# FoundationVision/OmniTokenizer

Measured on NVIDIA H100. Metric: video_frames_per_sec_encode_decode, higher is better.
Workload: dtype f32

## Files before the change

omnitokenizer_b200/csrc/attention_f16.cu:

```cuda
#include "omt_common.cuh"
#include "tc_ptx.cuh"
#include <cuda.h>

namespace omt {
int g_attn_f16_ctas = 2;
namespace af16 {
using namespace omt::ptx;

constexpr int QT = 128, KT = 64, D = 64;
constexpr int TILE = KT * D * 2;
constexpr int OFF_Q = 0;
constexpr int OFF_KV = 4 * TILE;
constexpr int OFF_P = OFF_KV + 8 * TILE;
constexpr int OFF_CTRL = OFF_P + 4 * TILE;
constexpr int SMEM = OFF_CTRL + 1024 + 1024;
constexpr int THREADS = 256;

struct Args {
  const float* vinv;
  long long rows;
  float* o; uint16_t* o_hi; uint16_t* o_lo; int ldo;
  int N;
  float scale_log2;
};

__global__ void __launch_bounds__(THREADS, 1)
attn_f16_kernel(const __grid_constant__ CUtensorMap tmQh, const __grid_constant__ CUtensorMap tmQl,
                const __grid_constant__ CUtensorMap tmKh, const __grid_constant__ CUtensorMap tmKl,
                const __grid_constant__ CUtensorMap tmVh, const __grid_constant__ CUtensorMap tmVl, const Args a) {
  extern __shared__ uint8_t smem_raw[];
  uint8_t* smem = smem_raw + ((1024u - (smem_u32(smem_raw) & 1023u)) & 1023u);
  uint64_t* bars = reinterpret_cast<uint64_t*>(smem + OFF_CTRL);
  uint64_t& q_full = bars[0];
  uint64_t* full = bars + 1;
  float* red = reinterpret_cast<float*>(smem + OFF_CTRL + 64);

  const int tid = threadIdx.x, warp = tid >> 5, lane = tid & 31;
  const int wg = warp >> 2, qd = lane & 3;
  const int qt = blockIdx.x, head = blockIdx.y, seq = blockIdx.z;
  const int ntiles = a.N / KT;
  const int row_q0 = seq * a.N + qt * QT;
  const int row_k0 = seq * a.N;
  const int col0 = head * D;

  if (tid == 0) {
    prefetch_map(&tmQh); prefetch_map(&tmQl); prefetch_map(&tmKh); prefetch_map(&tmKl); prefetch_map(&tmVh); prefetch_map(&tmVl);
    mbar_init(&q_full, 1); mbar_init(&full[0], 1); mbar_init(&full[1], 1);
    fence_barrier_init();
  }
  __syncthreads();
  pdl_sync();

  auto issue_kv = [&](int j) {
    const int s = j & 1;
    uint8_t* sp = smem + OFF_KV + s * 4 * TILE;
    const int kr = row_k0 + j * KT;
    mbar_expect_tx(&full[s], 4 * TILE);
    tma_load_2d(&tmKh, &full[s], sp, col0, kr);
    tma_load_2d(&tmKl, &full[s], sp + TILE, col0, kr);
    tma_load_2d(&tmVh, &full[s], sp + 2 * TILE, col0, kr);
    tma_load_2d(&tmVl, &full[s], sp + 3 * TILE, col0, kr);
  };
  if (tid == 0) {
    mbar_expect_tx(&q_full, 4 * TILE);
    for (int w = 0; w < 2; ++w) {
      tma_load_2d(&tmQh, &q_full, smem + OFF_Q + w * TILE, col0, row_q0 + w * 64);
      tma_load_2d(&tmQl, &q_full, smem + OFF_Q + (2 + w) * TILE, col0, row_q0 + w * 64);
    }
    issue_kv(0);
    if (ntiles > 1) issue_kv(1);
  }

  const float* vinv_h = a.vinv + (size_t)head * a.rows + row_k0;
  float vmx = 0.f;
  for (int i = tid; i < a.N; i += THREADS) vmx = fmaxf(vmx, __ldg(vinv_h + i));
  vmx = warp_max(vmx);
  if (lane == 0) red[warp] = vmx;
  __syncthreads();
#pragma unroll
  for (int i = 0; i < 8; ++i) vmx = fmaxf(vmx, red[i]);
  float p_scale, p_inv;
  row_scale(vmx, p_scale, p_inv);

  const uint32_t sb = smem_u32(smem);
  const uint64_t dq_hi = desc_sw128(sb + OFF_Q + wg * TILE), dq_lo = desc_sw128(sb + OFF_Q + (2 + wg) * TILE);
  const uint32_t p_hi = sb + OFF_P + wg * 2 * TILE, p_lo = p_hi + TILE;
  const uint64_t dp_hi = desc_sw128(p_hi), dp_lo = desc_sw128(p_lo);
  const int rl0 = (warp & 3) * 16 + (lane >> 2);
  float o_acc[32];
#pragma unroll
  for (int i = 0; i < 32; ++i) o_acc[i] = 0.f;
  float m_run[2] = {-INFINITY, -INFINITY}, l_run[2] = {0.f, 0.f};
  mbar_wait(&q_full, 0);

  for (int j = 0; j < ntiles; ++j) {
    const int s = j & 1;
    const uint32_t kv = sb + OFF_KV + s * 4 * TILE;
    mbar_wait(&full[s], (j >> 1) & 1);
    float sv[32];
    {
      const uint64_t dk_hi = desc_sw128(kv), dk_lo = desc_sw128(kv + TILE);
      wg_fence();
#pragma unroll
      for (int kk = 0; kk < 4; ++kk) {
        const uint64_t adv = (uint64_t)(kk * 2);
        wgmma_f16_n64(sv, dq_lo + adv, dk_hi + adv, kk != 0);
        wgmma_f16_n64(sv, dq_hi + adv, dk_lo + adv, 1);
        wgmma_f16_n64(sv, dq_hi + adv, dk_hi + adv, 1);
      }
      wg_commit();
      wg_wait<0>();
    }
    float alpha[2], nm[2];
#pragma unroll
    for (int h = 0; h < 2; ++h) {
      float mx = -INFINITY;
#pragma unroll
      for (int jj = 0; jj < 8; ++jj) mx = fmaxf(mx, fmaxf(sv[4 * jj + 2 * h], sv[4 * jj + 2 * h + 1]));
      mx = fmaxf(mx, __shfl_xor_sync(0xffffffffu, mx, 1));
      mx = fmaxf(mx, __shfl_xor_sync(0xffffffffu, mx, 2));
      const float m_new = fmaxf(m_run[h], mx);
      alpha[h] = ex2_fast((m_run[h] - m_new) * a.scale_log2);
      m_run[h] = m_new;
      nm[h] = -m_new;
    }
    const float* vi = vinv_h + j * KT;
    float ps[2] = {0.f, 0.f};
#pragma unroll
    for (int jj = 0; jj < 8; ++jj) {
      const int key = 8 * jj + 2 * qd;
      const float2 w = __ldg(reinterpret_cast<const float2*>(vi + key));
#pragma unroll
      for (int h = 0; h < 2; ++h) {
        const float e0 = ex2_fast((sv[4 * jj + 2 * h] + nm[h]) * a.scale_log2);
        const float e1 = ex2_fast((sv[4 * jj + 2 * h + 1] + nm[h]) * a.scale_log2);
        ps[h] += e0 + e1;
        uint32_t hw, lw;
        split2u(e0 * (w.x * p_scale), e1 * (w.y * p_scale), hw, lw);
        const int r = rl0 + 8 * h;
        const uint32_t off = (uint32_t)r * 128u + (uint32_t)((jj ^ (r & 7)) << 4) + (uint32_t)(qd * 4);
        asm volatile("st.shared.b32 [%0], %1;" ::"r"(p_hi + off), "r"(hw) : "memory");
        asm volatile("st.shared.b32 [%0], %1;" ::"r"(p_lo + off), "r"(lw) : "memory");
      }
    }
#pragma unroll
    for (int h = 0; h < 2; ++h) {
      l_run[h] = fmaf(l_run[h], alpha[h], ps[h]);
#pragma unroll
      for (int jj = 0; jj < 8; ++jj) { o_acc[4 * jj + 2 * h] *= alpha[h]; o_acc[4 * jj + 2 * h + 1] *= alpha[h]; }
    }
    fence_async_smem();
    wg_bar(1 + wg);
    {
      const uint32_t vh = kv + 2 * TILE, vl = kv + 3 * TILE;
      wg_fence();
#pragma unroll
      for (int kk = 0; kk < 4; ++kk) {
        const uint64_t adv = (uint64_t)(kk * 2);
        const uint64_t dvh = desc_sw128(vh + kk * 2048), dvl = desc_sw128(vl + kk * 2048);
        wgmma_f16_n64_tb(o_acc, dp_lo + adv, dvh, 1);
        wgmma_f16_n64_tb(o_acc, dp_hi + adv, dvl, 1);
        wgmma_f16_n64_tb(o_acc, dp_hi + adv, dvh, 1);
      }
      wg_commit();
      wg_wait<0>();
    }
    __syncthreads();
    if (tid == 0 && j + 2 < ntiles) issue_kv(j + 2);
  }
#pragma unroll
  for (int h = 0; h < 2; ++h) {
    float l = l_run[h];
    l += __shfl_xor_sync(0xffffffffu, l, 1);
    l += __shfl_xor_sync(0xffffffffu, l, 2);
    const float inv = p_inv / l;
    const size_t ooff = (size_t)(row_q0 + wg * 64 + rl0 + 8 * h) * a.ldo + col0 + 2 * qd;
#pragma unroll
    for (int jj = 0; jj < 8; ++jj) {
      const float2 ov = make_float2(o_acc[4 * jj + 2 * h] * inv, o_acc[4 * jj + 2 * h + 1] * inv);
      if (a.o_hi != nullptr) store_split2(a.o_hi, a.o_lo, ooff + 8 * jj, ov);
      else *reinterpret_cast<float2*>(a.o + ooff + 8 * jj) = ov;
    }
  }
}

typedef CUresult (*EncodeTiledFn)(CUtensorMap*, CUtensorMapDataType, cuuint32_t, void*, const cuuint64_t*,
                                  const cuuint64_t*, const cuuint32_t*, const cuuint32_t*, CUtensorMapInterleave,
                                  CUtensorMapSwizzle, CUtensorMapL2promotion, CUtensorMapFloatOOBfill);

static int encode2d(CUtensorMap* m, const uint16_t* base, int cols, long long rows, int ld) {
  static EncodeTiledFn fn = nullptr;
  if (fn == nullptr) {
    void* p = nullptr;
    cudaDriverEntryPointQueryResult qres;
    if (cudaGetDriverEntryPoint("cuTensorMapEncodeTiled", &p, cudaEnableDefault, &qres) == cudaSuccess &&
        qres == cudaDriverEntryPointSuccess)
      fn = reinterpret_cast<EncodeTiledFn>(p);
  }
  if (fn == nullptr) { set_error("cuTensorMapEncodeTiled entry point not found"); return OMT_E_CUDA; }
  cuuint64_t dims[2] = {(cuuint64_t)cols, (cuuint64_t)rows};
  cuuint64_t strides[1] = {(cuuint64_t)ld * 2};
  cuuint32_t box[2] = {64, (cuuint32_t)KT};
  cuuint32_t estr[2] = {1, 1};
  CUresult r = fn(m, CU_TENSOR_MAP_DATA_TYPE_FLOAT16, 2, const_cast<uint16_t*>(base), dims, strides, box, estr,
                  CU_TENSOR_MAP_INTERLEAVE_NONE, CU_TENSOR_MAP_SWIZZLE_128B, CU_TENSOR_MAP_L2_PROMOTION_L2_256B,
                  CU_TENSOR_MAP_FLOAT_OOB_FILL_NONE);
  if (r != CUDA_SUCCESS) { set_error("cuTensorMapEncodeTiled failed (%d)", (int)r); return OMT_E_CUDA; }
  return OMT_OK;
}

}
}

using namespace omt;

extern "C" int omt_attn_spatial_h(const uint16_t* q_hi, const uint16_t* q_lo, int ldq, const uint16_t* k_hi,
                                  const uint16_t* k_lo, int ldk, const uint16_t* v_hi, const uint16_t* v_lo, int ldv,
                                  const float* vinv, float qk_plane_scale, float* o, uint16_t* o_hi, uint16_t* o_lo, int ldo,
                                  int n_seq, int N, int heads, float scale, omt_stream_t stream) {
  using namespace af16;
  OMT_ENTER();
  OMT_REQUIRE(q_hi && q_lo && k_hi && k_lo && v_hi && v_lo && vinv && (o || o_hi) && ((o_hi == nullptr) == (o_lo == nullptr)),
              "omt_attn_spatial_h: null pointer");
  OMT_REQUIRE(N > 0 && N % QT == 0, "omt_attn_spatial_h: N=%d must be a multiple of 128", N);
  OMT_REQUIRE(ldq % 8 == 0 && ldk % 8 == 0 && ldv % 8 == 0 && ldo % 4 == 0, "omt_attn_spatial_h: bad leading dims");
  OMT_REQUIRE(((uintptr_t)q_hi | (uintptr_t)q_lo | (uintptr_t)k_hi | (uintptr_t)k_lo | (uintptr_t)v_hi | (uintptr_t)v_lo | (uintptr_t)vinv |
               (uintptr_t)o | (uintptr_t)o_hi | (uintptr_t)o_lo) % 16 == 0, "omt_attn_spatial_h: pointers must be 16-byte aligned");
  OMT_REQUIRE(heads > 0 && heads <= 65535 && n_seq <= 65535 && qk_plane_scale > 0.f, "omt_attn_spatial_h: bad arguments");
  if (n_seq == 0) return OMT_OK;
  const long long rows = (long long)n_seq * N;
  CUtensorMap tmQh, tmQl, tmKh, tmKl, tmVh, tmVl;
  int rc;
  if ((rc = encode2d(&tmQh, q_hi, heads * D, rows, ldq))) return rc;
  if ((rc = encode2d(&tmQl, q_lo, heads * D, rows, ldq))) return rc;
  if ((rc = encode2d(&tmKh, k_hi, heads * D, rows, ldk))) return rc;
  if ((rc = encode2d(&tmKl, k_lo, heads * D, rows, ldk))) return rc;
  if ((rc = encode2d(&tmVh, v_hi, heads * D, rows, ldv))) return rc;
  if ((rc = encode2d(&tmVl, v_lo, heads * D, rows, ldv))) return rc;
  static bool attr[64];
  int dev = 0;
  cudaGetDevice(&dev);
  if (dev >= 0 && dev < 64 && !attr[dev]) {
    OMT_CUDA(cudaFuncSetAttribute(attn_f16_kernel, cudaFuncAttributeMaxDynamicSharedMemorySize, SMEM));
    attr[dev] = true;
  }
  Args a{vinv, rows, o, o_hi, o_lo, ldo, N, scale * 1.4426950408889634f / qk_plane_scale};
  dim3 grid(N / QT, heads, n_seq);
  OMT_CUDA(launch_k(attn_f16_kernel, grid, dim3(THREADS), SMEM, (cudaStream_t)stream, tmQh, tmQl, tmKh, tmKl, tmVh, tmVl, a));
  OMT_LAUNCH_CHECK();
  return OMT_OK;
}
```

omnitokenizer_b200/csrc/tc_ptx.cuh:

```cuda
#pragma once
#include <cuda.h>
#include <cstdint>

namespace omt {
namespace ptx {

__device__ __forceinline__ uint32_t smem_u32(const void* p) { return static_cast<uint32_t>(__cvta_generic_to_shared(p)); }

__device__ __forceinline__ void mbar_init(uint64_t* bar, uint32_t count) {
  asm volatile("mbarrier.init.shared::cta.b64 [%0], %1;" ::"r"(smem_u32(bar)), "r"(count));
}
__device__ __forceinline__ void mbar_expect_tx(uint64_t* bar, uint32_t bytes) {
  asm volatile("mbarrier.arrive.expect_tx.shared::cta.b64 _, [%0], %1;" ::"r"(smem_u32(bar)), "r"(bytes) : "memory");
}
__device__ __forceinline__ void mbar_arrive(uint64_t* bar) {
  asm volatile("mbarrier.arrive.shared::cta.b64 _, [%0];" ::"r"(smem_u32(bar)) : "memory");
}
__device__ __forceinline__ void mbar_wait(uint64_t* bar, uint32_t parity) {
  const uint32_t addr = smem_u32(bar);
  const long long t0 = clock64();
  for (uint32_t it = 0;; ++it) {
    uint32_t ok;
    asm volatile(
        "{\n\t"
        ".reg .pred p;\n\t"
        "mbarrier.try_wait.parity.shared::cta.b64 p, [%1], %2;\n\t"
        "selp.b32 %0, 1, 0, p;\n\t"
        "}\n" : "=r"(ok) : "r"(addr), "r"(parity) : "memory");
    if (ok) break;
    if ((it & 0x3ff) == 0x3ff && clock64() - t0 > 4000000000LL) __trap();
  }
}
__device__ __forceinline__ void fence_barrier_init() { asm volatile("fence.mbarrier_init.release.cluster;" ::: "memory"); }

__device__ __forceinline__ uint32_t cluster_ctarank() { uint32_t r; asm volatile("mov.u32 %0, %%cluster_ctarank;" : "=r"(r)); return r; }
__device__ __forceinline__ uint32_t mapa(uint32_t addr, uint32_t rank) {
  uint32_t r;
  asm volatile("mapa.shared::cluster.u32 %0, %1, %2;" : "=r"(r) : "r"(addr), "r"(rank));
  return r;
}
__device__ __forceinline__ void cluster_arrive() { asm volatile("barrier.cluster.arrive.release.aligned;" ::: "memory"); }
__device__ __forceinline__ void cluster_wait() { asm volatile("barrier.cluster.wait.acquire.aligned;" ::: "memory"); }

template <uint32_t R> __device__ __forceinline__ void setmaxnreg_dec() { asm volatile("setmaxnreg.dec.sync.aligned.u32 %0;" ::"n"(R)); }
template <uint32_t R> __device__ __forceinline__ void setmaxnreg_inc() { asm volatile("setmaxnreg.inc.sync.aligned.u32 %0;" ::"n"(R)); }

__device__ __forceinline__ void tma_load_2d(const CUtensorMap* map, uint64_t* bar, void* dst, int c0, int c1) {
  asm volatile(
      "cp.async.bulk.tensor.2d.shared::cluster.global.tile.mbarrier::complete_tx::bytes [%0], [%1, {%3, %4}], [%2];"
      ::"r"(smem_u32(dst)), "l"(reinterpret_cast<uint64_t>(map)), "r"(smem_u32(bar)), "r"(c0), "r"(c1) : "memory");
}
__device__ __forceinline__ void tma_load_3d(const CUtensorMap* map, uint64_t* bar, void* dst, int c0, int c1, int c2) {
  asm volatile(
      "cp.async.bulk.tensor.3d.shared::cluster.global.tile.mbarrier::complete_tx::bytes [%0], [%1, {%3, %4, %5}], [%2];"
      ::"r"(smem_u32(dst)), "l"(reinterpret_cast<uint64_t>(map)), "r"(smem_u32(bar)), "r"(c0), "r"(c1), "r"(c2) : "memory");
}
__device__ __forceinline__ void prefetch_map(const CUtensorMap* map) {
  asm volatile("prefetch.tensormap [%0];" ::"l"(reinterpret_cast<uint64_t>(map)) : "memory");
}
__device__ __forceinline__ void fence_async_smem() { asm volatile("fence.proxy.async.shared::cta;" ::: "memory"); }
__device__ __forceinline__ void wg_bar(int id) { asm volatile("bar.sync %0, 128;" ::"r"(id) : "memory"); }
__device__ __forceinline__ void named_bar_sync(int id, int n) { asm volatile("bar.sync %0, %1;" ::"r"(id), "r"(n) : "memory"); }
__device__ __forceinline__ void named_bar_arrive(int id, int n) { asm volatile("bar.arrive %0, %1;" ::"r"(id), "r"(n) : "memory"); }

__device__ __forceinline__ float tf32_rn(float x) {
  return __uint_as_float((__float_as_uint(x) + 0x1000u) & 0xffffe000u);
}

__device__ __forceinline__ uint64_t desc_sw128(uint32_t saddr) {
  uint64_t d = 0;
  d |= (uint64_t)((saddr >> 4) & 0x3fff);
  d |= (uint64_t)1 << 16;
  d |= (uint64_t)(1024 >> 4) << 32;
  d |= (uint64_t)1 << 62;
  return d;
}
__device__ __forceinline__ void wg_fence() { asm volatile("wgmma.fence.sync.aligned;" ::: "memory"); }
__device__ __forceinline__ void wg_commit() { asm volatile("wgmma.commit_group.sync.aligned;" ::: "memory"); }
template <int N> __device__ __forceinline__ void wg_wait() { asm volatile("wgmma.wait_group.sync.aligned %0;" ::"n"(N) : "memory"); }

__device__ __forceinline__ void wgmma_tf32_n64(float (&d)[32], uint64_t da, uint64_t db, uint32_t scale_d) {
  asm volatile(
      "{\n\t.reg .pred p;\n\tsetp.ne.b32 p, %34, 0;\n\t"
      "wgmma.mma_async.sync.aligned.m64n64k8.f32.tf32.tf32 "
      "{%0, %1, %2, %3, %4, %5, %6, %7, %8, %9, %10, %11, %12, %13, %14, %15, %16, %17, %18, %19, %20, %21, %22, %23, %24, %25, %26, %27, %28, %29, %30, %31}, %32, %33, p, 1, 1;\n\t}\n"
      : "+f"(d[0]), "+f"(d[1]), "+f"(d[2]), "+f"(d[3]), "+f"(d[4]), "+f"(d[5]), "+f"(d[6]), "+f"(d[7]), "+f"(d[8]), "+f"(d[9]), "+f"(d[10]), "+f"(d[11]), "+f"(d[12]), "+f"(d[13]), "+f"(d[14]), "+f"(d[15]), "+f"(d[16]), "+f"(d[17]), "+f"(d[18]), "+f"(d[19]), "+f"(d[20]), "+f"(d[21]), "+f"(d[22]), "+f"(d[23]), "+f"(d[24]), "+f"(d[25]), "+f"(d[26]), "+f"(d[27]), "+f"(d[28]), "+f"(d[29]), "+f"(d[30]), "+f"(d[31])
      : "l"(da), "l"(db), "r"(scale_d));
}
__device__ __forceinline__ void wgmma_f16_n64(float (&d)[32], uint64_t da, uint64_t db, uint32_t scale_d) {
  asm volatile(
      "{\n\t.reg .pred p;\n\tsetp.ne.b32 p, %34, 0;\n\t"
      "wgmma.mma_async.sync.aligned.m64n64k16.f32.f16.f16 "
      "{%0, %1, %2, %3, %4, %5, %6, %7, %8, %9, %10, %11, %12, %13, %14, %15, %16, %17, %18, %19, %20, %21, %22, %23, %24, %25, %26, %27, %28, %29, %30, %31}, %32, %33, p, 1, 1, 0, 0;\n\t}\n"
      : "+f"(d[0]), "+f"(d[1]), "+f"(d[2]), "+f"(d[3]), "+f"(d[4]), "+f"(d[5]), "+f"(d[6]), "+f"(d[7]), "+f"(d[8]), "+f"(d[9]), "+f"(d[10]), "+f"(d[11]), "+f"(d[12]), "+f"(d[13]), "+f"(d[14]), "+f"(d[15]), "+f"(d[16]), "+f"(d[17]), "+f"(d[18]), "+f"(d[19]), "+f"(d[20]), "+f"(d[21]), "+f"(d[22]), "+f"(d[23]), "+f"(d[24]), "+f"(d[25]), "+f"(d[26]), "+f"(d[27]), "+f"(d[28]), "+f"(d[29]), "+f"(d[30]), "+f"(d[31])
      : "l"(da), "l"(db), "r"(scale_d));
}
__device__ __forceinline__ void wgmma_tf32_n128(float (&d)[64], uint64_t da, uint64_t db, uint32_t scale_d) {
  asm volatile(
      "{\n\t.reg .pred p;\n\tsetp.ne.b32 p, %66, 0;\n\t"
      "wgmma.mma_async.sync.aligned.m64n128k8.f32.tf32.tf32 "
      "{%0, %1, %2, %3, %4, %5, %6, %7, %8, %9, %10, %11, %12, %13, %14, %15, %16, %17, %18, %19, %20, %21, %22, %23, %24, %25, %26, %27, %28, %29, %30, %31, %32, %33, %34, %35, %36, %37, %38, %39, %40, %41, %42, %43, %44, %45, %46, %47, %48, %49, %50, %51, %52, %53, %54, %55, %56, %57, %58, %59, %60, %61, %62, %63}, %64, %65, p, 1, 1;\n\t}\n"
      : "+f"(d[0]), "+f"(d[1]), "+f"(d[2]), "+f"(d[3]), "+f"(d[4]), "+f"(d[5]), "+f"(d[6]), "+f"(d[7]), "+f"(d[8]), "+f"(d[9]), "+f"(d[10]), "+f"(d[11]), "+f"(d[12]), "+f"(d[13]), "+f"(d[14]), "+f"(d[15]), "+f"(d[16]), "+f"(d[17]), "+f"(d[18]), "+f"(d[19]), "+f"(d[20]), "+f"(d[21]), "+f"(d[22]), "+f"(d[23]), "+f"(d[24]), "+f"(d[25]), "+f"(d[26]), "+f"(d[27]), "+f"(d[28]), "+f"(d[29]), "+f"(d[30]), "+f"(d[31]), "+f"(d[32]), "+f"(d[33]), "+f"(d[34]), "+f"(d[35]), "+f"(d[36]), "+f"(d[37]), "+f"(d[38]), "+f"(d[39]), "+f"(d[40]), "+f"(d[41]), "+f"(d[42]), "+f"(d[43]), "+f"(d[44]), "+f"(d[45]), "+f"(d[46]), "+f"(d[47]), "+f"(d[48]), "+f"(d[49]), "+f"(d[50]), "+f"(d[51]), "+f"(d[52]), "+f"(d[53]), "+f"(d[54]), "+f"(d[55]), "+f"(d[56]), "+f"(d[57]), "+f"(d[58]), "+f"(d[59]), "+f"(d[60]), "+f"(d[61]), "+f"(d[62]), "+f"(d[63])
      : "l"(da), "l"(db), "r"(scale_d));
}
__device__ __forceinline__ void wgmma_f16_n128(float (&d)[64], uint64_t da, uint64_t db, uint32_t scale_d) {
  asm volatile(
      "{\n\t.reg .pred p;\n\tsetp.ne.b32 p, %66, 0;\n\t"
      "wgmma.mma_async.sync.aligned.m64n128k16.f32.f16.f16 "
      "{%0, %1, %2, %3, %4, %5, %6, %7, %8, %9, %10, %11, %12, %13, %14, %15, %16, %17, %18, %19, %20, %21, %22, %23, %24, %25, %26, %27, %28, %29, %30, %31, %32, %33, %34, %35, %36, %37, %38, %39, %40, %41, %42, %43, %44, %45, %46, %47, %48, %49, %50, %51, %52, %53, %54, %55, %56, %57, %58, %59, %60, %61, %62, %63}, %64, %65, p, 1, 1, 0, 0;\n\t}\n"
      : "+f"(d[0]), "+f"(d[1]), "+f"(d[2]), "+f"(d[3]), "+f"(d[4]), "+f"(d[5]), "+f"(d[6]), "+f"(d[7]), "+f"(d[8]), "+f"(d[9]), "+f"(d[10]), "+f"(d[11]), "+f"(d[12]), "+f"(d[13]), "+f"(d[14]), "+f"(d[15]), "+f"(d[16]), "+f"(d[17]), "+f"(d[18]), "+f"(d[19]), "+f"(d[20]), "+f"(d[21]), "+f"(d[22]), "+f"(d[23]), "+f"(d[24]), "+f"(d[25]), "+f"(d[26]), "+f"(d[27]), "+f"(d[28]), "+f"(d[29]), "+f"(d[30]), "+f"(d[31]), "+f"(d[32]), "+f"(d[33]), "+f"(d[34]), "+f"(d[35]), "+f"(d[36]), "+f"(d[37]), "+f"(d[38]), "+f"(d[39]), "+f"(d[40]), "+f"(d[41]), "+f"(d[42]), "+f"(d[43]), "+f"(d[44]), "+f"(d[45]), "+f"(d[46]), "+f"(d[47]), "+f"(d[48]), "+f"(d[49]), "+f"(d[50]), "+f"(d[51]), "+f"(d[52]), "+f"(d[53]), "+f"(d[54]), "+f"(d[55]), "+f"(d[56]), "+f"(d[57]), "+f"(d[58]), "+f"(d[59]), "+f"(d[60]), "+f"(d[61]), "+f"(d[62]), "+f"(d[63])
      : "l"(da), "l"(db), "r"(scale_d));
}
__device__ __forceinline__ void wgmma_f16_n64_tb(float (&d)[32], uint64_t da, uint64_t db, uint32_t scale_d) {
  asm volatile(
      "{\n\t.reg .pred p;\n\tsetp.ne.b32 p, %34, 0;\n\t"
      "wgmma.mma_async.sync.aligned.m64n64k16.f32.f16.f16 "
      "{%0, %1, %2, %3, %4, %5, %6, %7, %8, %9, %10, %11, %12, %13, %14, %15, %16, %17, %18, %19, %20, %21, %22, %23, %24, %25, %26, %27, %28, %29, %30, %31}, %32, %33, p, 1, 1, 0, 1;\n\t}\n"
      : "+f"(d[0]), "+f"(d[1]), "+f"(d[2]), "+f"(d[3]), "+f"(d[4]), "+f"(d[5]), "+f"(d[6]), "+f"(d[7]), "+f"(d[8]), "+f"(d[9]), "+f"(d[10]), "+f"(d[11]), "+f"(d[12]), "+f"(d[13]), "+f"(d[14]), "+f"(d[15]), "+f"(d[16]), "+f"(d[17]), "+f"(d[18]), "+f"(d[19]), "+f"(d[20]), "+f"(d[21]), "+f"(d[22]), "+f"(d[23]), "+f"(d[24]), "+f"(d[25]), "+f"(d[26]), "+f"(d[27]), "+f"(d[28]), "+f"(d[29]), "+f"(d[30]), "+f"(d[31])
      : "l"(da), "l"(db), "r"(scale_d));
}

}
}
```

Measured before the change: 3492.

## Warp-specialize attention into persistent producer/consumer pipeline with register-operand P

Rewrites the f16-split attention kernel as a persistent, warp-specialized design. One producer warpgroup issues TMA loads for Q, K, V and the vinv slice into a 4-stage mbarrier ring. Two consumer warpgroups keep Q and P in registers and use register-A wgmma, and they overlap the next tile's QK^T with the current PV product. This removes the per-tile __syncthreads, the shared-memory round trip for P, and the per-CTA launch/prologue cost. The cost is much more complex synchronization, register-budget pressure through setmaxnreg, and tail imbalance from the persistent grid.

After: 3603 (median of 6 runs). +3.2%, better.

```diff
diff --git a/omnitokenizer_b200/csrc/attention_f16.cu b/omnitokenizer_b200/csrc/attention_f16.cu
--- a/omnitokenizer_b200/csrc/attention_f16.cu
+++ b/omnitokenizer_b200/csrc/attention_f16.cu
@@ -9,18 +9,21 @@
 
 constexpr int QT = 128, KT = 64, D = 64;
 constexpr int TILE = KT * D * 2;
+constexpr int STAGES = 4;
 constexpr int OFF_Q = 0;
 constexpr int OFF_KV = 4 * TILE;
-constexpr int OFF_P = OFF_KV + 8 * TILE;
-constexpr int OFF_CTRL = OFF_P + 4 * TILE;
-constexpr int SMEM = OFF_CTRL + 1024 + 1024;
-constexpr int THREADS = 256;
+constexpr int OFF_VI = OFF_KV + STAGES * 4 * TILE;
+constexpr int OFF_CTRL = OFF_VI + STAGES * KT * 4;
+constexpr int SMEM = OFF_CTRL + 128 + 1024;
+constexpr int THREADS = 384;
+constexpr uint32_t KV_BYTES = 4 * TILE + KT * 4;
+constexpr int PRODUCER_REGS = 40, CONSUMER_REGS = 232;
 
 struct Args {
   const float* vinv;
   long long rows;
   float* o; uint16_t* o_hi; uint16_t* o_lo; int ldo;
-  int N;
+  int N, heads, items;
   float scale_log2;
 };
 
@@ -32,154 +35,224 @@
   uint8_t* smem = smem_raw + ((1024u - (smem_u32(smem_raw) & 1023u)) & 1023u);
   uint64_t* bars = reinterpret_cast<uint64_t*>(smem + OFF_CTRL);
   uint64_t& q_full = bars[0];
-  uint64_t* full = bars + 1;
-  float* red = reinterpret_cast<float*>(smem + OFF_CTRL + 64);
+  uint64_t& q_empty = bars[1];
+  uint64_t* full = bars + 2;
+  uint64_t* empty = full + STAGES;
+  float* vmax = reinterpret_cast<float*>(bars + 2 + 2 * STAGES);
 
   const int tid = threadIdx.x, warp = tid >> 5, lane = tid & 31;
-  const int wg = warp >> 2, qd = lane & 3;
-  const int qt = blockIdx.x, head = blockIdx.y, seq = blockIdx.z;
-  const int ntiles = a.N / KT;
-  const int row_q0 = seq * a.N + qt * QT;
-  const int row_k0 = seq * a.N;
-  const int col0 = head * D;
+  const int ntiles = a.N / KT, nqt = a.N / QT;
 
   if (tid == 0) {
     prefetch_map(&tmQh); prefetch_map(&tmQl); prefetch_map(&tmKh); prefetch_map(&tmKl); prefetch_map(&tmVh); prefetch_map(&tmVl);
-    mbar_init(&q_full, 1); mbar_init(&full[0], 1); mbar_init(&full[1], 1);
+    mbar_init(&q_full, 1);
+    mbar_init(&q_empty, 256);
+    for (int s = 0; s < STAGES; ++s) { mbar_init(&full[s], 1); mbar_init(&empty[s], 2); }
     fence_barrier_init();
   }
   __syncthreads();
   pdl_sync();
 
-  auto issue_kv = [&](int j) {
-    const int s = j & 1;
-    uint8_t* sp = smem + OFF_KV + s * 4 * TILE;
-    const int kr = row_k0 + j * KT;
-    mbar_expect_tx(&full[s], 4 * TILE);
-    tma_load_2d(&tmKh, &full[s], sp, col0, kr);
-    tma_load_2d(&tmKl, &full[s], sp + TILE, col0, kr);
-    tma_load_2d(&tmVh, &full[s], sp + 2 * TILE, col0, kr);
-    tma_load_2d(&tmVl, &full[s], sp + 3 * TILE, col0, kr);
+  auto decode = [&](int item, int& row_q0, int& row_k0, int& col0, int& head) {
+    const int qt = item % nqt, hs = item / nqt, seq = hs / a.heads;
+    head = hs % a.heads;
+    row_k0 = seq * a.N;
+    row_q0 = row_k0 + qt * QT;
+    col0 = head * D;
   };
-  if (tid == 0) {
-    mbar_expect_tx(&q_full, 4 * TILE);
-    for (int w = 0; w < 2; ++w) {
-      tma_load_2d(&tmQh, &q_full, smem + OFF_Q + w * TILE, col0, row_q0 + w * 64);
-      tma_load_2d(&tmQl, &q_full, smem + OFF_Q + (2 + w) * TILE, col0, row_q0 + w * 64);
+
+  if (warp < 4) {
+    setmaxnreg_dec<PRODUCER_REGS>();
+    if (warp == 0) {
+      uint32_t it = 0, c = 0;
+      for (int item = blockIdx.x; item < a.items; item += gridDim.x, ++c) {
+        int row_q0, row_k0, col0, head;
+        decode(item, row_q0, row_k0, col0, head);
+        const float* vinv_h = a.vinv + (size_t)head * a.rows + row_k0;
+        float vmx = 0.f;
+        for (int i = 4 * lane; i < a.N; i += 128) {
+          const float4 v = __ldg(reinterpret_cast<const float4*>(vinv_h + i));
+          vmx = fmaxf(vmx, fmaxf(fmaxf(v.x, v.y), fmaxf(v.z, v.w)));
+        }
+        vmx = warp_max(vmx);
+        mbar_wait(&q_empty, (c & 1) ^ 1);
+        if (lane == 0) {
+          *vmax = vmx;
+          mbar_expect_tx(&q_full, 4 * TILE);
+          for (int w = 0; w < 2; ++w) {
+            tma_load_2d(&tmQh, &q_full, smem + OFF_Q + w * TILE, col0, row_q0 + w * 64);
+            tma_load_2d(&tmQl, &q_full, smem + OFF_Q + (2 + w) * TILE, col0, row_q0 + w * 64);
+          }
+        }
+        for (int j = 0; j < ntiles; ++j, ++it) {
+          const int s = it % STAGES;
+          mbar_wait(&empty[s], ((it / STAGES) & 1) ^ 1);
+          if (lane == 0) {
+            uint8_t* sp = smem + OFF_KV + s * 4 * TILE;
+            const int kr = row_k0 + j * KT;
+            mbar_expect_tx(&full[s], KV_BYTES);
+            tma_load_2d(&tmKh, &full[s], sp, col0, kr);
+            tma_load_2d(&tmKl, &full[s], sp + TILE, col0, kr);
+            tma_load_2d(&tmVh, &full[s], sp + 2 * TILE, col0, kr);
+            tma_load_2d(&tmVl, &full[s], sp + 3 * TILE, col0, kr);
+            bulk_load(smem + OFF_VI + s * KT * 4, vinv_h + j * KT, KT * 4, &full[s]);
+          }
+        }
+      }
     }
-    issue_kv(0);
-    if (ntiles > 1) issue_kv(1);
-  }
-
-  const float* vinv_h = a.vinv + (size_t)head * a.rows + row_k0;
-  float vmx = 0.f;
-  for (int i = tid; i < a.N; i += THREADS) vmx = fmaxf(vmx, __ldg(vinv_h + i));
-  vmx = warp_max(vmx);
-  if (lane == 0) red[warp] = vmx;
-  __syncthreads();
-#pragma unroll
-  for (int i = 0; i < 8; ++i) vmx = fmaxf(vmx, red[i]);
-  float p_scale, p_inv;
-  row_scale(vmx, p_scale, p_inv);
-
-  const uint32_t sb = smem_u32(smem);
-  const uint64_t dq_hi = desc_sw128(sb + OFF_Q + wg * TILE), dq_lo = desc_sw128(sb + OFF_Q + (2 + wg) * TILE);
-  const uint32_t p_hi = sb + OFF_P + wg * 2 * TILE, p_lo = p_hi + TILE;
-  const uint64_t dp_hi = desc_sw128(p_hi), dp_lo = desc_sw128(p_lo);
-  const int rl0 = (warp & 3) * 16 + (lane >> 2);
-  float o_acc[32];
-#pragma unroll
-  for (int i = 0; i < 32; ++i) o_acc[i] = 0.f;
-  float m_run[2] = {-INFINITY, -INFINITY}, l_run[2] = {0.f, 0.f};
-  mbar_wait(&q_full, 0);
-
-  for (int j = 0; j < ntiles; ++j) {
-    const int s = j & 1;
-    const uint32_t kv = sb + OFF_KV + s * 4 * TILE;
-    mbar_wait(&full[s], (j >> 1) & 1);
+  } else {
+    setmaxnreg_inc<CONSUMER_REGS>();
+    const int wg = (warp >> 2) - 1, qd = lane & 3;
+    const int rl0 = (warp & 3) * 16 + (lane >> 2);
+    const uint32_t sb = smem_u32(smem);
+    auto release = [&](uint32_t t) {
+      if ((tid & 127) == 0) mbar_arrive(&empty[t % STAGES]);
+    };
     float sv[32];
-    {
-      const uint64_t dk_hi = desc_sw128(kv), dk_lo = desc_sw128(kv + TILE);
+#pragma unroll
+    for (int i = 0; i < 32; ++i) sv[i] = 0.f;
+    uint32_t it = 0, c = 0;
+    for (int item = blockIdx.x; item < a.items; item += gridDim.x, ++c) {
+      int row_q0, row_k0, col0, head;
+      decode(item, row_q0, row_k0, col0, head);
+      mbar_wait(&q_full, c & 1);
+      float p_scale, p_inv;
+      row_scale(*vmax, p_scale, p_inv);
+      uint32_t qh[16], ql[16];
+#pragma unroll
+      for (int kk = 0; kk < 4; ++kk)
+#pragma unroll
+        for (int e = 0; e < 2; ++e)
+#pragma unroll
+          for (int h = 0; h < 2; ++h) {
+            const int r = rl0 + 8 * h;
+            const uint8_t* p = smem + OFF_Q + wg * TILE + r * 128 + (((2 * kk + e) ^ (r & 7)) << 4) + qd * 4;
+            qh[4 * kk + 2 * e + h] = *reinterpret_cast<const uint32_t*>(p);
+            ql[4 * kk + 2 * e + h] = *reinterpret_cast<const uint32_t*>(p + 2 * TILE);
+          }
+      mbar_arrive(&q_empty);
+
+      float o_acc[32];
+#pragma unroll
+      for (int i = 0; i < 32; ++i) o_acc[i] = 0.f;
+      float m_run[2] = {-INFINITY, -INFINITY}, l_run[2] = {0.f, 0.f};
+      uint32_t p_a[2][16], p_b[2][16];
+      float alpha[2];
+
+      auto wait_full = [&](uint32_t t) { mbar_wait(&full[t % STAGES], (t / STAGES) & 1); };
+      auto issue_s = [&](uint32_t t) {
+        const uint32_t kv = sb + OFF_KV + (t % STAGES) * 4 * TILE;
+        const uint64_t dk_hi = desc_sw128(kv), dk_lo = desc_sw128(kv + TILE);
+#pragma unroll
+        for (int kk = 0; kk < 4; ++kk) {
+          const uint64_t adv = (uint64_t)(kk * 2);
+          wgmma_f16_n64_ra<0>(sv, ql + 4 * kk, dk_hi + adv, kk != 0);
+          wgmma_f16_n64_ra<0>(sv, qh + 4 * kk, dk_lo + adv, 1);
+          wgmma_f16_n64_ra<0>(sv, qh + 4 * kk, dk_hi + adv, 1);
+        }
+      };
+      auto issue_pv = [&](const uint32_t (&p)[2][16], uint32_t t) {
+        const uint32_t vh = sb + OFF_KV + (t % STAGES) * 4 * TILE + 2 * TILE, vl = vh + TILE;
+#pragma unroll
+        for (int kk = 0; kk < 4; ++kk) {
+          const uint64_t dvh = desc_sw128(vh + kk * 2048), dvl = desc_sw128(vl + kk * 2048);
+          wgmma_f16_n64_ra<1>(o_acc, p[1] + 4 * kk, dvh, 1);
+          wgmma_f16_n64_ra<1>(o_acc, p[0] + 4 * kk, dvl, 1);
+          wgmma_f16_n64_ra<1>(o_acc, p[0] + 4 * kk, dvh, 1);
+        }
+      };
+      auto softmax = [&](uint32_t (&p)[2][16], uint32_t t) {
+        float nm[2];
+#pragma unroll
+        for (int h = 0; h < 2; ++h) {
+          float mx = -INFINITY;
+#pragma unroll
+          for (int jj = 0; jj < 8; ++jj) mx = fmaxf(mx, fmaxf(sv[4 * jj + 2 * h], sv[4 * jj + 2 * h + 1]));
+          mx = fmaxf(mx, __shfl_xor_sync(0xffffffffu, mx, 1));
+          mx = fmaxf(mx, __shfl_xor_sync(0xffffffffu, mx, 2));
+          const float m_new = fmaxf(m_run[h], mx);
+          alpha[h] = ex2_fast((m_run[h] - m_new) * a.scale_log2);
+          m_run[h] = m_new;
+          nm[h] = -m_new;
+        }
+        const float* vi = reinterpret_cast<const float*>(smem + OFF_VI + (t % STAGES) * KT * 4);
+        float ps[2] = {0.f, 0.f};
+#pragma unroll
+        for (int jj = 0; jj < 8; ++jj) {
+          const float2 w = *reinterpret_cast<const float2*>(vi + 8 * jj + 2 * qd);
+#pragma unroll
+          for (int h = 0; h < 2; ++h) {
+            const float e0 = ex2_fast((sv[4 * jj + 2 * h] + nm[h]) * a.scale_log2);
+            const float e1 = ex2_fast((sv[4 * jj + 2 * h + 1] + nm[h]) * a.scale_log2);
+            ps[h] += e0 + e1;
+            const int wd = 4 * (jj >> 1) + 2 * (jj & 1) + h;
+            split2u(e0 * (w.x * p_scale), e1 * (w.y * p_scale), p[0][wd], p[1][wd]);
+          }
+        }
+#pragma unroll
+        for (int h = 0; h < 2; ++h) l_run[h] = fmaf(l_run[h], alpha[h], ps[h]);
+      };
+      auto rescale = [&]() {
+#pragma unroll
+        for (int h = 0; h < 2; ++h)
+#pragma unroll
+          for (int jj = 0; jj < 8; ++jj) { o_acc[4 * jj + 2 * h] *= alpha[h]; o_acc[4 * jj + 2 * h + 1] *= alpha[h]; }
+      };
+      auto step = [&](const uint32_t (&p)[2][16], uint32_t (&pn)[2][16], int j, bool next) {
+        const uint32_t t = it + j;
+        if (next) wait_full(t + 1);
+        reg_fence(sv);
+        reg_fence(o_acc);
+        wg_fence();
+        if (next) {
+          issue_s(t + 1);
+          wg_commit();
+        }
+        issue_pv(p, t);
+        wg_commit();
+        if (next) {
+          wg_wait<1>();
+          reg_fence(sv);
+          softmax(pn, t + 1);
+        }
+        wg_wait<0>();
+        reg_fence(o_acc);
+        release(t);
+        if (next) rescale();
+      };
+
+      wait_full(it);
+      reg_fence(sv);
       wg_fence();
-#pragma unroll
-      for (int kk = 0; kk < 4; ++kk) {
-        const uint64_t adv = (uint64_t)(kk * 2);
-        wgmma_f16_n64(sv, dq_lo + adv, dk_hi + adv, kk != 0);
-        wgmma_f16_n64(sv, dq_hi + adv, dk_lo + adv, 1);
-        wgmma_f16_n64(sv, dq_hi + adv, dk_hi + adv, 1);
-      }
+      issue_s(it);
       wg_commit();
       wg_wait<0>();
-    }
-    float alpha[2], nm[2];
-#pragma unroll
-    for (int h = 0; h < 2; ++h) {
-      float mx = -INFINITY;
-#pragma unroll
-      for (int jj = 0; jj < 8; ++jj) mx = fmaxf(mx, fmaxf(sv[4 * jj + 2 * h], sv[4 * jj + 2 * h + 1]));
-      mx = fmaxf(mx, __shfl_xor_sync(0xffffffffu, mx, 1));
-      mx = fmaxf(mx, __shfl_xor_sync(0xffffffffu, mx, 2));
-      const float m_new = fmaxf(m_run[h], mx);
-      alpha[h] = ex2_fast((m_run[h] - m_new) * a.scale_log2);
-      m_run[h] = m_new;
-      nm[h] = -m_new;
-    }
-    const float* vi = vinv_h + j * KT;
-    float ps[2] = {0.f, 0.f};
-#pragma unroll
-    for (int jj = 0; jj < 8; ++jj) {
-      const int key = 8 * jj + 2 * qd;
-      const float2 w = __ldg(reinterpret_cast<const float2*>(vi + key));
+      reg_fence(sv);
+      softmax(p_a, it);
+      rescale();
+      int j = 0;
+      for (; j + 2 < ntiles; j += 2) {
+        step(p_a, p_b, j, true);
+        step(p_b, p_a, j + 1, true);
+      }
+      step(p_a, p_b, j, true);
+      step(p_b, p_a, j + 1, false);
+      it += ntiles;
+
 #pragma unroll
       for (int h = 0; h < 2; ++h) {
-        const float e0 = ex2_fast((sv[4 * jj + 2 * h] + nm[h]) * a.scale_log2);
-        const float e1 = ex2_fast((sv[4 * jj + 2 * h + 1] + nm[h]) * a.scale_log2);
-        ps[h] += e0 + e1;
-        uint32_t hw, lw;
-        split2u(e0 * (w.x * p_scale), e1 * (w.y * p_scale), hw, lw);
-        const int r = rl0 + 8 * h;
-        const uint32_t off = (uint32_t)r * 128u + (uint32_t)((jj ^ (r & 7)) << 4) + (uint32_t)(qd * 4);
-        asm volatile("st.shared.b32 [%0], %1;" ::"r"(p_hi + off), "r"(hw) : "memory");
-        asm volatile("st.shared.b32 [%0], %1;" ::"r"(p_lo + off), "r"(lw) : "memory");
+        float l = l_run[h];
+        l += __shfl_xor_sync(0xffffffffu, l, 1);
+        l += __shfl_xor_sync(0xffffffffu, l, 2);
+        const float inv = p_inv / l;
+        const size_t ooff = (size_t)(row_q0 + wg * 64 + rl0 + 8 * h) * a.ldo + col0 + 2 * qd;
+#pragma unroll
+        for (int jj = 0; jj < 8; ++jj) {
+          const float2 ov = make_float2(o_acc[4 * jj + 2 * h] * inv, o_acc[4 * jj + 2 * h + 1] * inv);
+          if (a.o_hi != nullptr) store_split2(a.o_hi, a.o_lo, ooff + 8 * jj, ov);
+          else *reinterpret_cast<float2*>(a.o + ooff + 8 * jj) = ov;
+        }
       }
-    }
-#pragma unroll
-    for (int h = 0; h < 2; ++h) {
-      l_run[h] = fmaf(l_run[h], alpha[h], ps[h]);
-#pragma unroll
-      for (int jj = 0; jj < 8; ++jj) { o_acc[4 * jj + 2 * h] *= alpha[h]; o_acc[4 * jj + 2 * h + 1] *= alpha[h]; }
-    }
-    fence_async_smem();
-    wg_bar(1 + wg);
-    {
-      const uint32_t vh = kv + 2 * TILE, vl = kv + 3 * TILE;
-      wg_fence();
-#pragma unroll
-      for (int kk = 0; kk < 4; ++kk) {
-        const uint64_t adv = (uint64_t)(kk * 2);
-        const uint64_t dvh = desc_sw128(vh + kk * 2048), dvl = desc_sw128(vl + kk * 2048);
-        wgmma_f16_n64_tb(o_acc, dp_lo + adv, dvh, 1);
-        wgmma_f16_n64_tb(o_acc, dp_hi + adv, dvl, 1);
-        wgmma_f16_n64_tb(o_acc, dp_hi + adv, dvh, 1);
-      }
-      wg_commit();
-      wg_wait<0>();
-    }
-    __syncthreads();
-    if (tid == 0 && j + 2 < ntiles) issue_kv(j + 2);
-  }
-#pragma unroll
-  for (int h = 0; h < 2; ++h) {
-    float l = l_run[h];
-    l += __shfl_xor_sync(0xffffffffu, l, 1);
-    l += __shfl_xor_sync(0xffffffffu, l, 2);
-    const float inv = p_inv / l;
-    const size_t ooff = (size_t)(row_q0 + wg * 64 + rl0 + 8 * h) * a.ldo + col0 + 2 * qd;
-#pragma unroll
-    for (int jj = 0; jj < 8; ++jj) {
-      const float2 ov = make_float2(o_acc[4 * jj + 2 * h] * inv, o_acc[4 * jj + 2 * h + 1] * inv);
-      if (a.o_hi != nullptr) store_split2(a.o_hi, a.o_lo, ooff + 8 * jj, ov);
-      else *reinterpret_cast<float2*>(a.o + ooff + 8 * jj) = ov;
     }
   }
 }
@@ -229,6 +302,8 @@
   OMT_REQUIRE(heads > 0 && heads <= 65535 && n_seq <= 65535 && qk_plane_scale > 0.f, "omt_attn_spatial_h: bad arguments");
   if (n_seq == 0) return OMT_OK;
   const long long rows = (long long)n_seq * N;
+  const long long items = rows / QT * heads;
+  OMT_REQUIRE(rows < (1LL << 31) && items < (1LL << 31), "omt_attn_spatial_h: n_seq * N = %lld rows is too many", rows);
   CUtensorMap tmQh, tmQl, tmKh, tmKl, tmVh, tmVl;
   int rc;
   if ((rc = encode2d(&tmQh, q_hi, heads * D, rows, ldq))) return rc;
@@ -237,15 +312,20 @@
   if ((rc = encode2d(&tmKl, k_lo, heads * D, rows, ldk))) return rc;
   if ((rc = encode2d(&tmVh, v_hi, heads * D, rows, ldv))) return rc;
   if ((rc = encode2d(&tmVl, v_lo, heads * D, rows, ldv))) return rc;
-  static bool attr[64];
+  static int resident[64];
   int dev = 0;
-  cudaGetDevice(&dev);
-  if (dev >= 0 && dev < 64 && !attr[dev]) {
+  OMT_CUDA(cudaGetDevice(&dev));
+  OMT_REQUIRE(dev >= 0 && dev < 64, "omt_attn_spatial_h: device ordinal %d out of range", dev);
+  if (resident[dev] == 0) {
     OMT_CUDA(cudaFuncSetAttribute(attn_f16_kernel, cudaFuncAttributeMaxDynamicSharedMemorySize, SMEM));
-    attr[dev] = true;
+    int per_sm = 0, sms = 0;
+    OMT_CUDA(cudaOccupancyMaxActiveBlocksPerMultiprocessor(&per_sm, attn_f16_kernel, THREADS, SMEM));
+    OMT_CUDA(cudaDeviceGetAttribute(&sms, cudaDevAttrMultiProcessorCount, dev));
+    OMT_REQUIRE(per_sm > 0, "omt_attn_spatial_h: no CTA fits on an SM of device %d", dev);
+    resident[dev] = per_sm * sms;
   }
-  Args a{vinv, rows, o, o_hi, o_lo, ldo, N, scale * 1.4426950408889634f / qk_plane_scale};
-  dim3 grid(N / QT, heads, n_seq);
+  Args a{vinv, rows, o, o_hi, o_lo, ldo, N, heads, (int)items, scale * 1.4426950408889634f / qk_plane_scale};
+  const dim3 grid(items < resident[dev] ? (int)items : resident[dev]);
   OMT_CUDA(launch_k(attn_f16_kernel, grid, dim3(THREADS), SMEM, (cudaStream_t)stream, tmQh, tmQl, tmKh, tmKl, tmVh, tmVl, a));
   OMT_LAUNCH_CHECK();
   return OMT_OK;
diff --git a/omnitokenizer_b200/csrc/tc_ptx.cuh b/omnitokenizer_b200/csrc/tc_ptx.cuh
--- a/omnitokenizer_b200/csrc/tc_ptx.cuh
+++ b/omnitokenizer_b200/csrc/tc_ptx.cuh
@@ -54,6 +54,10 @@
   asm volatile(
       "cp.async.bulk.tensor.3d.shared::cluster.global.tile.mbarrier::complete_tx::bytes [%0], [%1, {%3, %4, %5}], [%2];"
       ::"r"(smem_u32(dst)), "l"(reinterpret_cast<uint64_t>(map)), "r"(smem_u32(bar)), "r"(c0), "r"(c1), "r"(c2) : "memory");
+}
+__device__ __forceinline__ void bulk_load(void* dst, const void* src, uint32_t bytes, uint64_t* bar) {
+  asm volatile("cp.async.bulk.shared::cluster.global.mbarrier::complete_tx::bytes [%0], [%1], %2, [%3];"
+               ::"r"(smem_u32(dst)), "l"(reinterpret_cast<uint64_t>(src)), "r"(bytes), "r"(smem_u32(bar)) : "memory");
 }
 __device__ __forceinline__ void prefetch_map(const CUtensorMap* map) {
   asm volatile("prefetch.tensormap [%0];" ::"l"(reinterpret_cast<uint64_t>(map)) : "memory");
@@ -119,6 +123,23 @@
       : "+f"(d[0]), "+f"(d[1]), "+f"(d[2]), "+f"(d[3]), "+f"(d[4]), "+f"(d[5]), "+f"(d[6]), "+f"(d[7]), "+f"(d[8]), "+f"(d[9]), "+f"(d[10]), "+f"(d[11]), "+f"(d[12]), "+f"(d[13]), "+f"(d[14]), "+f"(d[15]), "+f"(d[16]), "+f"(d[17]), "+f"(d[18]), "+f"(d[19]), "+f"(d[20]), "+f"(d[21]), "+f"(d[22]), "+f"(d[23]), "+f"(d[24]), "+f"(d[25]), "+f"(d[26]), "+f"(d[27]), "+f"(d[28]), "+f"(d[29]), "+f"(d[30]), "+f"(d[31])
       : "l"(da), "l"(db), "r"(scale_d));
 }
+template <int TB>
+__device__ __forceinline__ void wgmma_f16_n64_ra(float (&d)[32], const uint32_t* a, uint64_t db, uint32_t scale_d) {
+  asm volatile(
+      "{\n\t.reg .pred p;\n\tsetp.ne.b32 p, %38, 0;\n\t"
+      "wgmma.mma_async.sync.aligned.m64n64k16.f32.f16.f16 "
+      "{%0, %1, %2, %3, %4, %5, %6, %7, %8, %9, %10, %11, %12, %13, %14, %15, %16, %17, %18, %19, %20, %21, %22, %23, %24, %25, %26, %27, %28, %29, %30, %31}, {%32, %33, %34, %35}, %36, p, 1, 1, %37;\n\t}\n"
+      : "+f"(d[0]), "+f"(d[1]), "+f"(d[2]), "+f"(d[3]), "+f"(d[4]), "+f"(d[5]), "+f"(d[6]), "+f"(d[7]), "+f"(d[8]), "+f"(d[9]), "+f"(d[10]), "+f"(d[11]), "+f"(d[12]), "+f"(d[13]), "+f"(d[14]), "+f"(d[15]), "+f"(d[16]), "+f"(d[17]), "+f"(d[18]), "+f"(d[19]), "+f"(d[20]), "+f"(d[21]), "+f"(d[22]), "+f"(d[23]), "+f"(d[24]), "+f"(d[25]), "+f"(d[26]), "+f"(d[27]), "+f"(d[28]), "+f"(d[29]), "+f"(d[30]), "+f"(d[31])
+      : "r"(a[0]), "r"(a[1]), "r"(a[2]), "r"(a[3]), "l"(db), "n"(TB), "r"(scale_d));
+}
+template <int N> __device__ __forceinline__ void reg_fence(float (&r)[N]) {
+#pragma unroll
+  for (int i = 0; i < N; ++i) asm volatile("" : "+f"(r[i])::"memory");
+}
+template <int N> __device__ __forceinline__ void reg_fence(uint32_t (&r)[N]) {
+#pragma unroll
+  for (int i = 0; i < N; ++i) asm volatile("" : "+r"(r[i])::"memory");
+}
 
 }
 }
```
